# ICME-Lab/msm-webgpu

Measured on AMD Instinct MI355X. Metric: BN254 MSM/s at 2^20 points, higher is better.
Workload: dtype u32

## Files before the change

### include/msm_hip.h

```cpp
#ifndef MSM_HIP_H
#define MSM_HIP_H

#include <stddef.h>
#include <stdint.h>

#ifdef __cplusplus
extern "C" {
#endif

#define MSM_HIP_OK 0
#define MSM_HIP_ERR_NO_DEVICE (-1)
#define MSM_HIP_ERR_INVALID_ARG (-2)
#define MSM_HIP_ERR_OUT_OF_MEMORY (-3)
#define MSM_HIP_ERR_NONCANONICAL (-4)
#define MSM_HIP_ERR_NOT_ON_CURVE (-5)
#define MSM_HIP_ERR_NO_BASES (-6)
#define MSM_HIP_ERR_HIP (-7)
#define MSM_HIP_ERR_SLOT_BUSY (-8)

#define MSM_HIP_NUM_WINDOWS 16
#define MSM_HIP_WINDOW_BITS 16
#define MSM_HIP_MAX_LOCAL_WINDOWS 64
#define MSM_HIP_NUM_SLOTS 4
#define MSM_HIP_BUCKETS_PER_WINDOW 32768
// ... 103 lines not shown
int msm_hip_msm_bn254_g1(const uint8_t* xy_host, const uint8_t* scalars_host, size_t n, uint8_t out_xyz[96]);
int msm_hip_msm_curve(int curve, const uint8_t* xy_host, const uint8_t* scalars_host, size_t n, uint8_t* out_xyz);
void msm_hip_oneshot_release(void);

int msm_hip_sample_scalars_device(msm_hip_ctx* ctx, uint64_t seed, size_t n, void* scalars_dev);
int msm_hip_sample_points_device(msm_hip_ctx* ctx, uint64_t seed, size_t n, void* xy_dev);

int msm_hip_last_stage_ms(msm_hip_ctx* ctx, float* ms, int cap);
int msm_hip_set_stage_timing(msm_hip_ctx* ctx, int level);
void* msm_hip_stream(msm_hip_ctx* ctx);

#ifdef MSM_HIP_TEST_HOOKS
int msm_hip_set_debug(msm_hip_ctx* ctx, int keep_digit_planes);
int msm_hip_set_fine_hist_min_n(msm_hip_ctx* ctx, size_t n);
int msm_hip_test_skew_credit(const msm_hip_ctx* ctx);
int msm_hip_test_env_report(const msm_hip_ctx* ctx, char* out, size_t cap);
int msm_hip_read_digits(msm_hip_ctx* ctx, uint16_t* out, size_t cap_elems);
int msm_hip_read_col_ptr(msm_hip_ctx* ctx, uint32_t* out, size_t cap_elems);
int msm_hip_read_val_idxs(msm_hip_ctx* ctx, uint32_t* out, size_t cap_elems);
int msm_hip_read_buckets(msm_hip_ctx* ctx, uint8_t* out, size_t cap_bytes);
int msm_hip_read_window_sums(msm_hip_ctx* ctx, uint8_t* out, size_t cap_bytes);

int msm_hip_test_fq_op(msm_hip_ctx* ctx, int op, const uint8_t* a, const uint8_t* b, uint8_t* out, size_t n);
int msm_hip_test_g1_op(msm_hip_ctx* ctx, int op, const uint8_t* a, const uint8_t* b, uint8_t* out, size_t n);
int msm_hip_test_g1_mul_u32(msm_hip_ctx* ctx, const uint8_t* a, const uint32_t* k, uint8_t* out, size_t n);

int msm_hip_mgpu_inject_fault(msm_hip_mgpu* m, int device_index, int launches);

int msm_hip_test_oneshot_parts(int parts, size_t min_points);
#endif
// ... 33 lines not shown
```

### msm-webgpu_amd/api.py

```python
import ctypes as C
import os

import numpy as np
import torch

from . import build as _build

P = 21888242871839275222246405745257275088696311157297823662689037894645226208583
R_BN254 = 21888242871839275222246405745257275088548364400416034343698204186575808495617
PALLAS_P = 0x40000000000000000000000000000000224698fc094cf91b992d30ed00000001
VESTA_P = 0x40000000000000000000000000000000224698fc0994a8dd8c46eb2100000001
BLS12_381_P = 0x1a0111ea397fe69a4b1ba7b6434bacd764774b84f38512bf6730d2a0f6b0f6241eabfffeb153ffffb9feffffffffaaab
CURVES = {"bn254": (0, P), "grumpkin": (1, R_BN254), "pallas": (2, PALLAS_P), "vesta": (3, VESTA_P), "bls12_381": (4, BLS12_381_P),
          "bn254_g2": (5, P), "bls12_381_g2": (6, BLS12_381_P)}


def coord_bytes(curve):
    return {"bls12_381": 48, "bn254_g2": 64, "bls12_381_g2": 96}.get(curve, 32)
NUM_WINDOWS = 16
WINDOW_BITS = 16
BUCKETS_PER_WINDOW = 1 << 15

_lib = None

# ... 49 lines not shown
        L.msm_hip_slot_sync.argtypes = [vp, i]
        L.msm_hip_combine_windows_bn254.argtypes = [u8p, i, u8p]
        L.msm_hip_msm_bn254_g1.argtypes = [u8p, u8p, sz, u8p]
        L.msm_hip_msm_curve.argtypes = [i, u8p, u8p, sz, u8p]
        L.msm_hip_test_oneshot_parts.argtypes = [i, sz]
        L.msm_hip_oneshot_release.argtypes = []
        L.msm_hip_oneshot_release.restype = None
        L.msm_hip_sample_scalars_device.argtypes = [vp, C.c_uint64, sz, vp]
        L.msm_hip_sample_points_device.argtypes = [vp, C.c_uint64, sz, vp]
        L.msm_hip_last_stage_ms.argtypes = [vp, C.POINTER(C.c_float), i]
        L.msm_hip_stream.argtypes = [vp]
        L.msm_hip_stream.restype = vp
        L.msm_hip_set_debug.argtypes = [vp, i]
        L.msm_hip_set_fine_hist_min_n.argtypes = [vp, sz]
        L.msm_hip_test_skew_credit.argtypes = [vp]
        L.msm_hip_test_env_report.argtypes = [vp, C.c_char_p, sz]
        L.msm_hip_set_scalar_format.argtypes = [vp, C.c_uint32]
        L.msm_hip_set_stage_timing.argtypes = [vp, i]
        L.msm_hip_set_window_bits.argtypes = [vp, i]
        L.msm_hip_set_wide_bits.argtypes = [vp, i]
        L.msm_hip_wide_bits.argtypes = [vp]
        L.msm_hip_wide_config.argtypes = [i, i, C.c_size_t] + [C.POINTER(C.c_int)] * 4
        L.msm_hip_window_config.argtypes = [i, C.POINTER(i), C.POINTER(i)]
        L.msm_hip_last_window_bits.argtypes = [vp]
        L.msm_hip_endomorphism_window_count.argtypes = [i]
        L.msm_hip_uses_endomorphism.argtypes = [vp]
        L.msm_hip_batch_group_size.argtypes = [vp, sz]
        L.msm_hip_read_digits.argtypes = [vp, vp, sz]
        L.msm_hip_read_col_ptr.argtypes = [vp, vp, sz]
        L.msm_hip_read_val_idxs.argtypes = [vp, vp, sz]
# ... 455 lines not shown
        if mont256 and width != 32:
            raise ValueError("mont256 scalars are 32 bytes wide")
        fmt = SCALAR_WIDTHS[width] if width != 32 else (1 if mont256 else 0)
        _check(lib().msm_hip_set_scalar_format(self._h, fmt), "msm_hip_set_scalar_format")
        self.scalar_width = width

    def skew_credit(self):
        return lib().msm_hip_test_skew_credit(self._h)

    def env_report(self):
        return env_report(self._h)

    def set_fine_hist_min_n(self, n):
        _check(lib().msm_hip_set_fine_hist_min_n(self._h, n), "msm_hip_set_fine_hist_min_n")

    def set_debug(self, keep_digit_planes=True):
        _check(lib().msm_hip_set_debug(self._h, 1 if keep_digit_planes else 0), "msm_hip_set_debug")

    def read_digits(self, n, w_count=NUM_WINDOWS):
        a = np.empty((w_count, n), dtype=np.uint16)
        _check(lib().msm_hip_read_digits(self._h, a.ctypes.data, a.size), "msm_hip_read_digits")
        return a

    def read_col_ptr(self, w_count=NUM_WINDOWS, buckets=BUCKETS_PER_WINDOW):
        a = np.empty((w_count, buckets + 1), dtype=np.uint32)
        _check(lib().msm_hip_read_col_ptr(self._h, a.ctypes.data, a.size), "msm_hip_read_col_ptr")
        return a

    def read_val_idxs(self, n, w_count=NUM_WINDOWS):
        a = np.empty((w_count, n), dtype=np.uint32)
# ... 172 lines not shown
```

### msm-webgpu_amd/csrc/msm_hip.hip

```cpp
#include <hip/hip_runtime.h>
#include <hip/hip_ext.h>

#include <algorithm>
#include <chrono>
#include <cmath>
#include <cstdio>
#include <cstdlib>
#include <cstring>
#include <mutex>
#include <new>
#include <type_traits>

#define MSM_HIP_TEST_HOOKS 1
#include "../../include/msm_hip.h"
#include "curve_ops.h"
#include "host_pool.h"

#define MSM_FIELD_NS bn254
#define MSM_KERNEL_NS msmk
#define MSM_CURVE_CONSTANTS "bn254_constants.h"
#include "curve_unit.h"
#undef MSM_FIELD_NS
#undef MSM_KERNEL_NS
#undef MSM_CURVE_CONSTANTS
// ... 47 lines not shown
  bool pairs = false;
  uint32_t* sums_dev = nullptr;
  int wbits = WBITS;
  uint32_t half = 0, ncoarse = 0;
  int w_count = 0;
  int nwin = 0, combine_bits = 0;
  bool whole = false;
  size_t n_sc = 0, n_entries = 0;
  int full_windows = 0;
  bool digits = false;
  bool planes = false, share_shape = false, list_path = false;
  uint32_t tiles = 0, tile_len = 0, subtiles = 0;
  uint32_t chunks = 0, chunk_len = 0;
  size_t stride = 0;
  bool sparse = false;
  const uint32_t* indices = nullptr;
};

struct Slot {
  uint8_t* h_wsums = nullptr;
  uint8_t* d_wsums = nullptr;
  uint32_t* d_buckets = nullptr;
  size_t cap_buckets = 0;
  uint32_t* d_partials = nullptr;
  uint32_t* d_col_ptr = nullptr;
  uint32_t* d_heads = nullptr;
  uint32_t* d_tails = nullptr;
  uint32_t* d_big_queue = nullptr;
  hipEvent_t ev[N_MAIN_EVENTS] = {};
  hipEvent_t red0 = nullptr, red1 = nullptr;
// ... 69 lines not shown
  uint32_t* d_bin_total = nullptr;
  uint32_t* d_coarse_ptr = nullptr;
  uint32_t* d_tmp_val = nullptr;
  uint8_t* d_tmp_fine = nullptr;
  uint32_t* d_val = nullptr;
  uint32_t* d_chunk_slot = nullptr;
  uint32_t* d_list_len = nullptr;
  size_t cap_list_len = 0;
  uint32_t* d_scalar_conv = nullptr;
  size_t cap_scalar_conv = 0;
  uint32_t scalar_format = 0;
  int window_bits = 0;
  uint32_t* d_part_hist = nullptr;
  size_t fine_hist_min_n = FINE_BIG + 1;
  int skew_credit = 0;
  uint32_t* d_err = nullptr;
  uint8_t* d_stage = nullptr;
  size_t cap_stage = 0;

  Slot slot[NSLOT];
  LaunchPlan last;
  int last_slot = 0;
  int last_logr = 0;
  bool last_inline_reduce = false;
  bool last_fine_hist = false;
  bool sort_fine_hist = false;
  float stage_ms[10] = {};
};

namespace {
// ... 377 lines not shown
  p.tile_len = 2048;
  if ((p.n_sc + p.tile_len - 1) / p.tile_len > MAX_TILES) p.tile_len = (uint32_t)((((p.n_sc + MAX_TILES - 1) / MAX_TILES) + tile_unit - 1) / tile_unit * tile_unit);
  p.tiles = (uint32_t)((p.n_sc + p.tile_len - 1) / p.tile_len);
  p.subtiles = (uint32_t)((p.n_sc + LIST_SUB - 1) / LIST_SUB);
  if (wide) {
    const WideShape ws = wide_shape(n, ctx->curve, ctx->wide_bits, w_count);
    p.chunk_len = ws.host_len;
    p.chunks = ws.chunks;
  } else {
    p.chunk_len = chunk_len_for(p.n_entries, w_count);
    p.chunks = chunks_for(p.n_entries, p.chunk_len);
  }
  p.stride = stride_for(p.n_entries);
  p.sparse = sparse;
  p.indices = indices;
  return MSM_HIP_OK;
}

template <auto V0, auto... Vs, typename F>
void dispatch(decltype(V0) v, F&& f) {
  if constexpr (sizeof...(Vs) == 0) f(std::integral_constant<decltype(V0), V0>{});
  else if (v == V0) f(std::integral_constant<decltype(V0), V0>{});
  else dispatch<Vs...>(v, f);
}

int enqueue_sort(msm_hip_ctx* ctx, const LaunchPlan& p, Slot& s, const uint32_t* d_scalars) {
  const bool merge = p.mode == MODE_TABLES, halves = p.mode == MODE_HALVES, wide = p.mode == MODE_WIDE;
  const bool bytes = byte_windows(p.nb);
  const size_t merge_nb = merge || wide ? ctx->n_bases : 0;
  hipStream_t st = ctx->stream;
// ... 79 lines not shown
    });
  } else if (p.planes) {
    hipLaunchKernelGGL(k_scatter_planes, dim3(p.tiles), dim3(256), 0, st, ctx->d_digits, halves ? ctx->d_negbits : (const uint64_t*)nullptr, p.n_sc, p.stride,
                       p.tile_len, p.tiles, p.w_count, p.w_count_vec, ctx->d_counts, ctx->d_bin_total, ctx->d_coarse_ptr, ctx->d_tmp_val, ctx->d_tmp_fine,
                       (uint32_t)ctx->n_bases, p.chunks, p.chunk_len, d_chunk_len);
  } else if (bytes) {
    dispatch<1, 2>(p.nb, [&](auto b) {
      if (p.sparse)
        hipLaunchKernelGGL((k_byte_scatter<decltype(b)::value, SparseIdx>), grid, block, 0, st, (const uint8_t*)d_scalars, p.n, p.stride, p.tile_len, p.tiles,
                           p.w_count, ctx->d_counts, ctx->d_bin_total, s.d_col_ptr, p.half, ctx->d_val, p.chunks, p.chunk_len, d_chunk_len, sp);
      else
        hipLaunchKernelGGL(k_byte_scatter<decltype(b)::value>, grid, block, 0, st, (const uint8_t*)d_scalars, p.n, p.stride, p.tile_len, p.tiles, p.w_count,
                           ctx->d_counts, ctx->d_bin_total, s.d_col_ptr, p.half, ctx->d_val, p.chunks, p.chunk_len, d_chunk_len);
    });
  } else {
    dispatch<16, 14, 12>(p.wbits, [&](auto c) {
      dispatch<8, 4, 2, 1>(sw, [&](auto w) {
        constexpr int C = decltype(c)::value, SW = decltype(w)::value, NB = SW < 4 ? 4 * SW : 0;
        if (p.sparse)
          hipLaunchKernelGGL((k_scatter_coarse<C, SW, NB, SparseIdx>), grid, block, gpos_bytes, st, d_scalars, p.n_sc, p.stride, p.tile_len, p.tiles, p.w_begin,
                             p.w_count_vec, p.nvec, p.n * (NB ? NB : 8), ctx->d_counts, ctx->d_bin_total, ctx->d_coarse_ptr, ctx->d_tmp_val, ctx->d_tmp_fine,
                             merge_nb, (uint32_t)p.n, halves ? (uint32_t)ctx->n_bases : 0u, p.chunks, p.chunk_len, d_chunk_len, sp);
        else
          hipLaunchKernelGGL((k_scatter_coarse<C, SW, NB>), grid, block, gpos_bytes, st, d_scalars, p.n_sc, p.stride, p.tile_len, p.tiles, p.w_begin,
                             p.w_count_vec, p.nvec, p.n * (NB ? NB : 8), ctx->d_counts, ctx->d_bin_total, ctx->d_coarse_ptr, ctx->d_tmp_val, ctx->d_tmp_fine,
                             merge_nb, (uint32_t)p.n, halves ? (uint32_t)ctx->n_bases : 0u, p.chunks, p.chunk_len, d_chunk_len);
      });
    });
  }
  AFTER_KERNEL(ctx, "k_scatter_coarse", st);
  HIP_TRY(ctx, mark(3));
  if (bytes) {
    hipLaunchKernelGGL(k_byte_chunks, dim3(blocks_for(p.chunks, 256), p.w_count), dim3(256), 0, st, (const uint32_t*)s.d_col_ptr, p.half, p.chunks,
                       (const uint32_t*)d_chunk_len, ctx->d_chunk_slot);
    AFTER_KERNEL(ctx, "k_byte_chunks", st);
  } else {
    const uint32_t* part_hist = nullptr;
    const bool hist_useful = p.nb || ctx->fine_hist_min_n != FINE_BIG + 1 || p.n_entries / p.ncoarse * 4 > (size_t)FINE_BIG * 3 || ctx->skew_credit > 0;
    if (ctx->skew_credit > 0 && !p.nb) ctx->skew_credit--;
    ctx->sort_fine_hist = p.n_entries >= ctx->fine_hist_min_n && hist_useful;
    if (ctx->sort_fine_hist) {
      hipLaunchKernelGGL(k_fine_hist, dim3(p.ncoarse, p.w_count, FINE_SPLIT), dim3(256), 0, st, ctx->d_tmp_fine, p.stride, ctx->d_coarse_ptr,
                         ctx->d_part_hist);
      AFTER_KERNEL(ctx, "k_fine_hist", st);
      part_hist = ctx->d_part_hist;
    }
    hipLaunchKernelGGL(k_sort_fine, dim3(p.ncoarse, p.w_count, FINE_SPLIT), dim3(256), 0, st, ctx->d_tmp_val, ctx->d_tmp_fine, p.stride, ctx->d_coarse_ptr,
                       s.d_col_ptr, ctx->d_val, p.chunks, d_chunk_len, ctx->d_chunk_slot, part_hist, d_err);
    AFTER_KERNEL(ctx, "k_sort_fine", st);
  }
  if (ctx->debug) {
    hipLaunchKernelGGL(k_order_runs, dim3(blocks_for(p.n_entries, 256), p.w_count), dim3(256), 0, st, s.d_col_ptr, ctx->d_val, ctx->d_tmp_val, p.stride, p.half);
    hipLaunchKernelGGL(k_copy_runs, dim3(blocks_for(p.n_entries, 256), p.w_count), dim3(256), 0, st, s.d_col_ptr, ctx->d_tmp_val, ctx->d_val, p.stride, p.half);
    AFTER_KERNEL(ctx, "k_order_runs", st);
  }
  return MSM_HIP_OK;
}

struct RowCol {
  void (*kernel)(const uint32_t*, uint32_t*, uint32_t*);
  int blocks;
  int logr;
};
// ... 1012 lines not shown

int msm_hip_uses_endomorphism(const msm_hip_ctx* ctx) { return ctx ? (ctx->endo ? 1 : 0) : MSM_HIP_ERR_INVALID_ARG; }

int msm_hip_batch_group_size(msm_hip_ctx* ctx, size_t n) {
  if (!ctx) return MSM_HIP_ERR_INVALID_ARG;
  return (int)batch_group(ctx, n, (size_t)MAXLW);
}

int msm_hip_set_fine_hist_min_n(msm_hip_ctx* ctx, size_t n) {
  if (!ctx) return MSM_HIP_ERR_INVALID_ARG;
  ctx->fine_hist_min_n = n;
  return MSM_HIP_OK;
}

int msm_hip_test_skew_credit(const msm_hip_ctx* ctx) { return ctx ? ctx->skew_credit : MSM_HIP_ERR_INVALID_ARG; }

int msm_hip_test_env_report(const msm_hip_ctx* ctx, char* out, size_t cap) {
  if (!out || !cap) return MSM_HIP_ERR_INVALID_ARG;
  size_t len = 0;
  bool fits = true;
  auto put = [&](const char* key, long long v) {
    const int w = snprintf(out + len, cap - len, "%s=%lld\n", key, v);
    if (w < 0 || (size_t)w >= cap - len) fits = false;
    else len += (size_t)w;
  };
  put("target_lanes", (long long)target_lanes());
  put("chunk_search", chunk_search());
  put("window_bits", env_window_bits());
  put("bpr_logr", bpr_force_logr());
  put("planes_max_w", planes_max_w());
// ... 16 lines not shown
  put("upload_parts", g_probe_upload_parts.load());
  put("upload_chunks", g_probe_upload_chunks.load());
  if (ctx) {
    put("fine_hist_min_n", (long long)ctx->fine_hist_min_n);
    put("last_wbits", ctx->last.wbits);
    put("last_chunk_len", ctx->last.chunk_len);
    put("last_chunks", ctx->last.chunks);
    put("last_planes", ctx->last.planes);
    put("last_list_path", ctx->last.list_path);
    put("last_mode", ctx->last.mode);
    put("last_w_count", ctx->last.w_count);
    put("last_wide_top_shift", ctx->last.mode == MODE_WIDE ? wide_top_shift(ctx->curve, ctx->last.wide_bits) : 0);
    put("last_logr", ctx->last_logr);
    put("last_inline_reduce", ctx->last_inline_reduce);
    put("last_fine_hist", ctx->last_fine_hist);
  }
  return fits ? (int)len : MSM_HIP_ERR_INVALID_ARG;
}

int msm_hip_set_debug(msm_hip_ctx* ctx, int keep_digit_planes) {
  if (!ctx) return MSM_HIP_ERR_INVALID_ARG;
  ctx->debug = keep_digit_planes != 0;
  return MSM_HIP_OK;
}

int msm_hip_read_digits(msm_hip_ctx* ctx, uint16_t* out, size_t cap_elems) {
  if (!ctx || !ctx->last.digits) return MSM_HIP_ERR_INVALID_ARG;
  return read_back(ctx, out, ctx->d_digits, ctx->last.n_sc * ctx->last.w_count * 2, cap_elems * 2);
}
int msm_hip_read_col_ptr(msm_hip_ctx* ctx, uint32_t* out, size_t cap_elems) {
// ... 154 lines not shown
```

### msm-webgpu_amd/csrc/msm_kernels.h

```cpp
#ifndef MSM_CURVE_UNIT
#pragma once
#include "g1.h"
#endif
#include <hip/hip_runtime.h>

#include <utility>

#ifndef MSM_SPARSE_IDX
#define MSM_SPARSE_IDX
struct SparseIdx {
  const uint32_t* idx;
  uint32_t n_bases;
  uint32_t* err;
};
#endif

namespace MSM_KERNEL_NS {
using namespace MSM_FIELD_NS;

constexpr int WBITS = 16;
constexpr int NWIN = 16;
constexpr int MAXLW = 64;
constexpr int HALF = 1 << (WBITS - 1);
constexpr int CW = FQ_WORDS;
// ... 198 lines not shown
  for (int w = 1; w < num_tables; w++) {
    const int steps = w == num_tables - 1 ? last_step_bits : step_bits;
#pragma unroll 1
    for (int k = 0; k < steps; k++) acc = g1_double(acc);
    const fq t = fq_inv(fq_mul(acc.zz, acc.zzz));
    const fq x = fq_canonical(fq_mul(acc.x, fq_mul(t, acc.zzz)));
    const fq y = fq_canonical(fq_mul(acc.y, fq_mul(t, acc.zz)));
    st_fq(bases + ((size_t)w * nb + i) * PT_WORDS, x);
    st_fq(bases + ((size_t)w * nb + i) * PT_WORDS + CW, y);
    acc = g1_from_affine(x, y);
  }
}

constexpr int NCOARSE = 128;
constexpr int FINE = HALF / NCOARSE;

template <int C, int SW = 8, int NB = 0>
__host__ __device__ constexpr uint32_t bias_word(int i) {
  uint32_t v = 0;
  for (int w = 0; w < WinCfg<C, SW, NB>::NWIN; w++) {
    const int bit = C * w + C - 1;
    if (bit / 32 == i) v |= 1u << (bit % 32);
  }
  return v;
}
template <int C, int SW = 8, int NB = 0>
__device__ __forceinline__ uint32_t bias_scalar(const uint32_t s[SW], uint32_t t[WinCfg<C, SW, NB>::WORDS]) {
  constexpr int WORDS = WinCfg<C, SW, NB>::WORDS;
  uint64_t c = 0;
#pragma unroll
// ... 91 lines not shown
}

__global__ void __launch_bounds__(256) k_scalars_from_mont256(const uint32_t* __restrict__ in, uint32_t* __restrict__ out, size_t count,
                                                              uint32_t* __restrict__ err) {
  const size_t i = (size_t)blockIdx.x * blockDim.x + threadIdx.x;
  if (i >= count) return;
  uint32_t w[8], o[8];
  ld8(in + i * 8, w);
  if (geq_modulus<1>(w)) atomicOr(err, ERRBIT_NONCANONICAL);
  fr_from_mont256(w, o);
  uint4* q = reinterpret_cast<uint4*>(out + i * 8);
  q[0] = make_uint4(o[0], o[1], o[2], o[3]);
  q[1] = make_uint4(o[4], o[5], o[6], o[7]);
}

__device__ __forceinline__ SparseIdx sparse_arg() { return SparseIdx{nullptr, 0u, nullptr}; }
__device__ __forceinline__ SparseIdx sparse_arg(SparseIdx s) { return s; }
template <int C, int SW, bool SPLIT = false, int NB = 0, typename... Sparse>
__global__ void __launch_bounds__(256) k_count(const uint32_t* __restrict__ scalars, size_t n, uint32_t tile_len, uint32_t tiles,
                                               int w_begin, int w_count, int nvec, size_t vec_stride,
                                               uint32_t* __restrict__ counts, uint16_t* __restrict__ planes, int plane_mode,
                                               uint64_t* __restrict__ negbits, uint32_t* __restrict__ halves_out,
                                               uint32_t* __restrict__ err, size_t merge_nb, Sparse... sparse) {
  static_assert(!SPLIT || SW == 4, "the split produces 4-word halves");
  static_assert(!SPLIT || NB == 0, "narrow scalars are never split");
  constexpr bool SPARSE = sizeof...(Sparse) != 0;
  const SparseIdx sp = sparse_arg(sparse...);
  uint32_t bad_idx = 0;
  __shared__ uint32_t cnt[MAXLW * NCOARSE];
  const int tid = threadIdx.x;
  const int v = blockIdx.y;
  const int le0 = merge_nb ? v : v * w_count, le_n = merge_nb ? 1 : w_count;
  (void)nvec;
  for (int i = tid; i < le_n * NCOARSE; i += 256) cnt[le0 * NCOARSE + i] = 0;
// ... 5 lines not shown
#pragma unroll
    for (int w = 0; w < WinCfg<C, SW, NB>::NWIN; w++) {
      const int lw = w - w_begin;
      if (lw >= 0 && lw < w_count) {
        const int le = merge_nb ? v : v * w_count + lw;
        const uint32_t code = code_of_window<C>(tb, w);
        if (code != 0) atomicAdd(&cnt[le * NCOARSE + ((code & 0x7fffu) >> 8)], 1u);
        if (plane_mode) planes[((size_t)v * w_count + lw) * n + pos] = (uint16_t)(plane_mode == 2 ? code : (code ? code ^ (neg << 15) : 0u));
      }
    }
  };
  {
    const uint32_t* sv = scalars + (size_t)v * vec_stride;
    if constexpr (SPLIT) {
      const size_t nsc = n / 2, neg_words = (nsc + 63) / 64;
      for (size_t j0 = base / 2; j0 < end / 2; j0 += 256) {
        const size_t j = j0 + tid;
        const bool valid = j < end / 2;
        uint32_t k[8], h[2][4];
#pragma unroll
        for (int q = 0; q < 8; q++) k[q] = 0;
        bool live = valid;
        if constexpr (SPARSE) {
          if (valid && sp.idx[j] >= sp.n_bases) live = false, bad_idx = 1;
        }
        if (live) ld8(sv + j * 8, k);
        uint64_t c = 0;
#pragma unroll
        for (int q = 0; q < 8; q++) c = (c + k[q] + 0x80008000u) >> 32;
        const bool ok = glv_split(k, h[0], h[1]);
        if (c != 0 || !ok) bad = 1;
        if (negbits) {
#pragma unroll
          for (int hh = 0; hh < 2; hh++) {
            const unsigned long long nb = __ballot((h[hh][3] >> 31) != 0u);
            if ((tid & 63) == 0 && valid) negbits[((size_t)v * 2 + hh) * neg_words + j / 64] = nb;
          }
        }
        if (!valid) continue;
        if (halves_out) {
          uint4* o = reinterpret_cast<uint4*>(halves_out + ((size_t)v * nsc + j) * 8);
          o[0] = make_uint4(h[0][0], h[0][1], h[0][2], h[0][3]);
          o[1] = make_uint4(h[1][0], h[1][1], h[1][2], h[1][3]);
        }
#pragma unroll
        for (int hh = 0; hh < 2; hh++) {
          uint32_t s[4] = {h[hh][0], h[hh][1], h[hh][2], h[hh][3] & 0x7fffffffu}, tb[WinCfg<C, 4>::WORDS];
          bad |= bias_scalar<C, 4>(s, tb);
          emit(v, 2 * j + hh, tb, h[hh][3] >> 31);
        }
      }
    } else if constexpr (NB != 0) {
      const uint8_t* nv = reinterpret_cast<const uint8_t*>(scalars) + (size_t)v * vec_stride;
      for (size_t i0 = base; i0 < end; i0 += 256) {
        const size_t i = i0 + tid;
        if (i >= end) continue;
        uint32_t s[SW], tb[WinCfg<C, SW, NB>::WORDS];
        ld_narrow<NB>(nv, i, s);
        if constexpr (SPARSE) {
          if (sp.idx[i] >= sp.n_bases) {
            bad_idx = 1;
#pragma unroll
            for (int k = 0; k < SW; k++) s[k] = 0;
          }
// ... 21 lines not shown
          bad |= bias_scalar<16>(s, t16);
        }
        emit(v, i, tb, neg);
      }
    }
  }
  if (bad) atomicOr(err, ERRBIT_SCALAR_CARRY);
  if constexpr (SPARSE) {
    if (bad_idx) atomicOr(err, ERRBIT_BAD_INDEX);
  }
  __syncthreads();
  for (int i = tid; i < le_n * NCOARSE; i += 256)
    counts[((size_t)(le0 + i / NCOARSE) * tiles + blockIdx.x) * NCOARSE + (i % NCOARSE)] = cnt[le0 * NCOARSE + i];
}

__global__ void __launch_bounds__(256) k_scan_tiles(uint32_t* __restrict__ counts, uint32_t tiles, uint32_t* __restrict__ bin_total) {
  const int lw = blockIdx.y, lane = threadIdx.x & 63;
  const int bin = blockIdx.x * 4 + (threadIdx.x >> 6);
  uint32_t* c = counts + (size_t)lw * tiles * NCOARSE + bin;
  uint32_t run = 0;
  for (uint32_t t0 = 0; t0 < tiles; t0 += 64) {
    const uint32_t t = t0 + lane;
    const uint32_t v = t < tiles ? c[(size_t)t * NCOARSE] : 0u;
    uint32_t x = v;
#pragma unroll
    for (int off = 1; off < 64; off <<= 1) {
      const uint32_t y = __shfl_up(x, off);
      if (lane >= off) x += y;
    }
    if (t < tiles) c[(size_t)t * NCOARSE] = run + x - v;
    run += __shfl(x, 63);
  }
  if (lane == 0) bin_total[lw * NCOARSE + bin] = run;
}

__device__ __forceinline__ uint32_t block_excl_scan_256(uint32_t v, uint32_t* wave_tot) {
  const int lane = threadIdx.x & 63, wid = threadIdx.x >> 6;
  uint32_t x = v;
#pragma unroll
  for (int off = 1; off < 64; off <<= 1) {
    const uint32_t y = __shfl_up(x, off);
    if (lane >= off) x += y;
  }
  if (lane == 63) wave_tot[wid] = x;
  __syncthreads();
// ... 109 lines not shown
      __syncthreads();
      const uint32_t mine = tid < NCOARSE ? hist[tid] : 0u;
      const uint32_t excl = block_excl_scan_256(mine, wave_tot);
      if (tid < NCOARSE) lstart[tid] = excl;
      __syncthreads();
      const uint32_t total = lstart[NCOARSE - 1] + hist[NCOARSE - 1];
#pragma unroll
      for (int j = 0; j < PER; j++) {
        const uint32_t code = code_of_window<C>(sc[j], w);
        if (code) {
          const uint32_t slot = code & 0x7fffu, bin = slot >> 8;
          const uint32_t e = lstart[bin] + rank[j];
          uint32_t pos = (uint32_t)(sub + (size_t)j * 256 + tid);
          if constexpr (SPARSE) pos = rec[j];
          else if constexpr (SW == 4) pos = (pos >> 1) + ((pos & 1u) ? half_shift : 0u);
          st_val[e] = (idx_base + pos) | (((code >> 15) ^ ((negs >> j) & 1u)) << 31);
          st_fine[e] = (uint8_t)(slot & 0xffu);
          st_dst[e] = gpos[lw * NCOARSE + bin] + rank[j];
        }
      }
      __syncthreads();
      uint32_t* ov = tmp_val + (size_t)lw * stride;
      uint8_t* of = tmp_fine + (size_t)lw * stride;
      for (uint32_t e = tid; e < total; e += 256) {
        const uint32_t d = st_dst[e];
        ov[d] = st_val[e];
        of[d] = st_fine[e];
      }
      if (tid < NCOARSE) gpos[lw * NCOARSE + tid] += hist[tid];
      __syncthreads();
    }
  }
}

constexpr int BYTE_BINS = 256;
constexpr int BYTE_MAXLW = MAXLW * NCOARSE / BYTE_BINS;
template <int NB>
__device__ __forceinline__ uint32_t ld_byte_scalar(const uint8_t* v, size_t i) {
  static_assert(NB == 1 || NB == 2, "byte windows: U8 / U16");
  if constexpr (NB == 1) return v[i];
  else return reinterpret_cast<const uint16_t*>(v)[i];
}
// ... 750 lines not shown
  const unsigned long long vm = __ballot(valid);
  if (vm == 0) return;
  const int first = __ffsll((long long)vm) - 1;
  const uint32_t k0 = (uint32_t)__builtin_amdgcn_readlane((int)key, first);
  const bool same = valid && key == k0;
  const unsigned long long sm = __ballot(same);
  if ((int)(threadIdx.x & 63) == first) atomicAdd(&counter[k0], (uint32_t)__popcll(sm));
  if (valid && !same) atomicAdd(&counter[key], 1u);
}

constexpr int FINE_SPLIT = 8;

constexpr uint32_t FINE_BIG = 32768;
static_assert(FINE_BIG % FINE_CHUNK == 0, "sub-ranges are whole chunks");

__global__ void __launch_bounds__(256) k_fine_hist(const uint8_t* __restrict__ tmp_fine, size_t stride,
                                                   const uint32_t* __restrict__ coarse_ptr, uint32_t* __restrict__ part_hist) {
  __shared__ uint32_t hist[FINE];
  const int bin = blockIdx.x, part = blockIdx.z, lw = blockIdx.y, tid = threadIdx.x;
  const uint32_t begin = coarse_ptr[(size_t)lw * (NCOARSE + 1) + bin], end = coarse_ptr[(size_t)lw * (NCOARSE + 1) + bin + 1];
  if (end - begin <= FINE_BIG) return;
  uint32_t per = (end - begin + FINE_SPLIT - 1) / FINE_SPLIT;
  per = (per + FINE_CHUNK - 1) / FINE_CHUNK * FINE_CHUNK;
  const uint32_t my_begin = begin + (uint32_t)part * per < end ? begin + (uint32_t)part * per : end;
  const uint32_t my_end = my_begin + per < end ? my_begin + per : end;
  const uint8_t* tf = tmp_fine + (size_t)lw * stride;
  hist[tid] = 0;
  __syncthreads();
  for (uint32_t base = my_begin; base < my_end; base += FINE_CHUNK) {
    uint32_t f[FINE_PER];
#pragma unroll
    for (int j = 0; j < FINE_PER; j++) {
      const uint32_t i = base + j * 256 + tid;
      f[j] = i < my_end ? tf[i] : 0xffffffffu;
    }
#pragma unroll
    for (int j = 0; j < FINE_PER; j++) lds_count_only(hist, f[j] & 0xffu, f[j] != 0xffffffffu);
  }
  __syncthreads();
  part_hist[(((size_t)lw * NCOARSE + bin) * FINE_SPLIT + part) * FINE + tid] = hist[tid];
}

__global__ void __launch_bounds__(256) k_sort_fine(const uint32_t* __restrict__ tmp_val, const uint8_t* __restrict__ tmp_fine, size_t stride,
                                                   const uint32_t* __restrict__ coarse_ptr, uint32_t* __restrict__ col_ptr,
                                                   uint32_t* __restrict__ val_idxs, uint32_t chunks, const uint32_t* __restrict__ chunk_len_dev,
                                                   uint32_t* __restrict__ chunk_slot, const uint32_t* __restrict__ part_hist, uint32_t* __restrict__ info) {
  const uint32_t chunk_len = *chunk_len_dev;
  __shared__ uint32_t hist[FINE];
  __shared__ uint32_t before[FINE];
  __shared__ uint32_t lstart[FINE];
  __shared__ uint32_t gpos[FINE];
  __shared__ uint32_t wave_tot[4];
  __shared__ uint32_t st_val[FINE_CHUNK];
  __shared__ uint8_t st_slot[FINE_CHUNK];
  __shared__ uint32_t long_c0[FINE], long_c1[FINE], long_slot[FINE];
  __shared__ uint32_t skew_flag, long_count;
  const int bin = blockIdx.x, part = blockIdx.z, lw = blockIdx.y, tid = threadIdx.x;
  const uint32_t half = gridDim.x * FINE;
  const uint32_t begin = coarse_ptr[(size_t)lw * (NCOARSE + 1) + bin], end = coarse_ptr[(size_t)lw * (NCOARSE + 1) + bin + 1];
  const bool big = end - begin > FINE_BIG;
  if (!big && part != 0) return;
  uint32_t my_begin = begin, my_end = end;
  if (big) {
    uint32_t per = (end - begin + FINE_SPLIT - 1) / FINE_SPLIT;
    per = (per + FINE_CHUNK - 1) / FINE_CHUNK * FINE_CHUNK;
    my_begin = begin + (uint32_t)part * per < end ? begin + (uint32_t)part * per : end;
    my_end = my_begin + per < end ? my_begin + per : end;
  }
  const uint32_t* tv = tmp_val + (size_t)lw * stride;
  const uint8_t* tf = tmp_fine + (size_t)lw * stride;
  uint32_t* out = val_idxs + (size_t)lw * stride;
  hist[tid] = 0;
  before[tid] = 0;
  if (tid == 0) {
    skew_flag = 0;
    long_count = 0;
  }
  __syncthreads();
  if (!big) {
    for (uint32_t base = begin; base < end; base += FINE_CHUNK) {
      uint32_t f[FINE_PER];
#pragma unroll
      for (int j = 0; j < FINE_PER; j++) {
        const uint32_t i = base + j * 256 + tid;
        f[j] = i < end ? tf[i] : 0xffffffffu;
      }
#pragma unroll
      for (int j = 0; j < FINE_PER; j++)
        if (f[j] != 0xffffffffu) atomicAdd(&hist[f[j]], 1u);
    }
  } else if (part_hist) {
    if (tid == 0 && part == 0) atomicOr(info, INFOBIT_HUGE_BIN);
    const uint32_t* ph = part_hist + ((size_t)lw * NCOARSE + bin) * FINE_SPLIT * FINE + tid;
    uint32_t all = 0, front = 0;
#pragma unroll
    for (int q = 0; q < FINE_SPLIT; q++) {
      const uint32_t c = ph[q * FINE];
      all += c;
      if (q < part) front += c;
    }
    hist[tid] = all;
    before[tid] = front;
  } else {
    if (tid == 0 && part == 0) atomicOr(info, INFOBIT_HUGE_BIN);
    uint32_t f[FINE_PER], g[FINE_PER];
#pragma unroll
    for (int j = 0; j < FINE_PER; j++) {
      const uint32_t i = begin + j * 256 + tid;
      f[j] = i < end ? tf[i] : 0xffffffffu;
    }
    for (uint32_t base = begin; base < end; base += FINE_CHUNK) {
#pragma unroll
      for (int j = 0; j < FINE_PER; j++) {
        const uint32_t i = base + FINE_CHUNK + j * 256 + tid;
        g[j] = i < end ? tf[i] : 0xffffffffu;
      }
      uint32_t* counter = base < my_begin ? before : hist;
#pragma unroll
      for (int j = 0; j < FINE_PER; j++) lds_count_only(counter, f[j] & 0xffu, f[j] != 0xffffffffu);
#pragma unroll
      for (int j = 0; j < FINE_PER; j++) f[j] = g[j];
    }
    __syncthreads();
    hist[tid] += before[tid];
  }
  __syncthreads();
  if (hist[tid] > (end - begin) / 4 && end - begin > (uint32_t)FINE_CHUNK) skew_flag = 1;
  {
    const uint32_t excl = block_excl_scan_256(hist[tid], wave_tot);
    gpos[tid] = begin + excl + before[tid];
// ... 20 lines not shown
  {
    const uint32_t nl = long_count, nparts = big ? FINE_SPLIT : 1;
    for (uint32_t k = 0; k < nl; k++)
      for (uint32_t c = long_c0[k] + part * 256 + tid; c < long_c1[k]; c += nparts * 256) chunk_slot[(size_t)lw * chunks + c] = long_slot[k];
  }
  __syncthreads();
  const bool skewed = skew_flag != 0;
  for (uint32_t base = my_begin; base < my_end; base += FINE_CHUNK) {
    hist[tid] = 0;
    __syncthreads();
    uint32_t v[FINE_PER], fr[FINE_PER];
#pragma unroll
    for (int j = 0; j < FINE_PER; j++) {
      const uint32_t i = base + j * 256 + tid;
      const bool valid = i < my_end;
      const uint32_t f = valid ? tf[i] : 0u;
      const uint32_t rank = skewed ? lds_count_rank(hist, f, valid) : (valid ? atomicAdd(&hist[f], 1u) : 0u);
      if (valid) {
        v[j] = tv[i];
        fr[j] = f | (rank << 8);
      } else {
        fr[j] = 0xffffffffu;
      }
    }
    __syncthreads();
    const uint32_t excl = block_excl_scan_256(hist[tid], wave_tot);
    lstart[tid] = excl;
    __syncthreads();
    const uint32_t total = (my_end - base) < (uint32_t)FINE_CHUNK ? (my_end - base) : (uint32_t)FINE_CHUNK;
#pragma unroll
    for (int j = 0; j < FINE_PER; j++) {
      if (fr[j] != 0xffffffffu) {
        const uint32_t f = fr[j] & 0xffu, r = fr[j] >> 8;
        const uint32_t e = lstart[f] + r;
// ... 1011 lines not shown
```

Baseline: 736.5.

## Pack fine bucket key into value word; prefetch in split count and scan

```diff
diff --git a/include/msm_hip.h b/include/msm_hip.h
--- a/include/msm_hip.h
+++ b/include/msm_hip.h
@@ -141,6 +141,7 @@
 int msm_hip_set_debug(msm_hip_ctx* ctx, int keep_digit_planes);
 int msm_hip_set_fine_hist_min_n(msm_hip_ctx* ctx, size_t n);
 int msm_hip_test_skew_credit(const msm_hip_ctx* ctx);
+int msm_hip_test_pack_fine(msm_hip_ctx* ctx, int allow);
 int msm_hip_test_env_report(const msm_hip_ctx* ctx, char* out, size_t cap);
 int msm_hip_read_digits(msm_hip_ctx* ctx, uint16_t* out, size_t cap_elems);
 int msm_hip_read_col_ptr(msm_hip_ctx* ctx, uint32_t* out, size_t cap_elems);
diff --git a/msm-webgpu_amd/api.py b/msm-webgpu_amd/api.py
--- a/msm-webgpu_amd/api.py
+++ b/msm-webgpu_amd/api.py
@@ -87,6 +87,7 @@
         L.msm_hip_set_debug.argtypes = [vp, i]
         L.msm_hip_set_fine_hist_min_n.argtypes = [vp, sz]
         L.msm_hip_test_skew_credit.argtypes = [vp]
+        L.msm_hip_test_pack_fine.argtypes = [vp, i]
         L.msm_hip_test_env_report.argtypes = [vp, C.c_char_p, sz]
         L.msm_hip_set_scalar_format.argtypes = [vp, C.c_uint32]
         L.msm_hip_set_stage_timing.argtypes = [vp, i]
@@ -572,6 +573,9 @@
     def set_fine_hist_min_n(self, n):
         _check(lib().msm_hip_set_fine_hist_min_n(self._h, n), "msm_hip_set_fine_hist_min_n")
 
+    def set_pack_fine(self, allow=True):
+        _check(lib().msm_hip_test_pack_fine(self._h, 1 if allow else 0), "msm_hip_test_pack_fine")
+
     def set_debug(self, keep_digit_planes=True):
         _check(lib().msm_hip_set_debug(self._h, 1 if keep_digit_planes else 0), "msm_hip_set_debug")
 
diff --git a/msm-webgpu_amd/csrc/msm_hip.hip b/msm-webgpu_amd/csrc/msm_hip.hip
--- a/msm-webgpu_amd/csrc/msm_hip.hip
+++ b/msm-webgpu_amd/csrc/msm_hip.hip
@@ -85,6 +85,7 @@
   uint32_t chunks = 0, chunk_len = 0;
   size_t stride = 0;
   bool sparse = false;
+  bool packed = false;
   const uint32_t* indices = nullptr;
 };
 
@@ -184,6 +185,7 @@
   uint32_t* d_part_hist = nullptr;
   size_t fine_hist_min_n = FINE_BIG + 1;
   int skew_credit = 0;
+  bool pack_fine = true;
   uint32_t* d_err = nullptr;
   uint8_t* d_stage = nullptr;
   size_t cap_stage = 0;
@@ -591,6 +593,8 @@
   p.stride = stride_for(p.n_entries);
   p.sparse = sparse;
   p.indices = indices;
+  const size_t rec_bound = merge ? (size_t)(w_begin + w_count_vec) * ctx->n_bases : halves ? 2 * ctx->n_bases : ctx->n_bases;
+  p.packed = ctx->pack_fine && !wide && !p.planes && !byte_windows(nb) && rec_bound <= ((size_t)1 << FINE_KEY_SHIFT);
   return MSM_HIP_OK;
 }
 
@@ -700,16 +704,17 @@
                            ctx->d_counts, ctx->d_bin_total, s.d_col_ptr, p.half, ctx->d_val, p.chunks, p.chunk_len, d_chunk_len);
     });
   } else {
+    uint8_t* tmp_fine = p.packed ? nullptr : ctx->d_tmp_fine;
     dispatch<16, 14, 12>(p.wbits, [&](auto c) {
       dispatch<8, 4, 2, 1>(sw, [&](auto w) {
         constexpr int C = decltype(c)::value, SW = decltype(w)::value, NB = SW < 4 ? 4 * SW : 0;
         if (p.sparse)
           hipLaunchKernelGGL((k_scatter_coarse<C, SW, NB, SparseIdx>), grid, block, gpos_bytes, st, d_scalars, p.n_sc, p.stride, p.tile_len, p.tiles, p.w_begin,
-                             p.w_count_vec, p.nvec, p.n * (NB ? NB : 8), ctx->d_counts, ctx->d_bin_total, ctx->d_coarse_ptr, ctx->d_tmp_val, ctx->d_tmp_fine,
+                             p.w_count_vec, p.nvec, p.n * (NB ? NB : 8), ctx->d_counts, ctx->d_bin_total, ctx->d_coarse_ptr, ctx->d_tmp_val, tmp_fine,
                              merge_nb, (uint32_t)p.n, halves ? (uint32_t)ctx->n_bases : 0u, p.chunks, p.chunk_len, d_chunk_len, sp);
         else
           hipLaunchKernelGGL((k_scatter_coarse<C, SW, NB>), grid, block, gpos_bytes, st, d_scalars, p.n_sc, p.stride, p.tile_len, p.tiles, p.w_begin,
-                             p.w_count_vec, p.nvec, p.n * (NB ? NB : 8), ctx->d_counts, ctx->d_bin_total, ctx->d_coarse_ptr, ctx->d_tmp_val, ctx->d_tmp_fine,
+                             p.w_count_vec, p.nvec, p.n * (NB ? NB : 8), ctx->d_counts, ctx->d_bin_total, ctx->d_coarse_ptr, ctx->d_tmp_val, tmp_fine,
                              merge_nb, (uint32_t)p.n, halves ? (uint32_t)ctx->n_bases : 0u, p.chunks, p.chunk_len, d_chunk_len);
       });
     });
@@ -726,13 +731,14 @@
     if (ctx->skew_credit > 0 && !p.nb) ctx->skew_credit--;
     ctx->sort_fine_hist = p.n_entries >= ctx->fine_hist_min_n && hist_useful;
     if (ctx->sort_fine_hist) {
-      hipLaunchKernelGGL(k_fine_hist, dim3(p.ncoarse, p.w_count, FINE_SPLIT), dim3(256), 0, st, ctx->d_tmp_fine, p.stride, ctx->d_coarse_ptr,
-                         ctx->d_part_hist);
+      hipLaunchKernelGGL(p.packed ? k_fine_hist<true> : k_fine_hist<false>, dim3(p.ncoarse, p.w_count, FINE_SPLIT), dim3(256), 0, st,
+                         (const uint32_t*)ctx->d_tmp_val, (const uint8_t*)ctx->d_tmp_fine, p.stride, (const uint32_t*)ctx->d_coarse_ptr, ctx->d_part_hist);
       AFTER_KERNEL(ctx, "k_fine_hist", st);
       part_hist = ctx->d_part_hist;
     }
-    hipLaunchKernelGGL(k_sort_fine, dim3(p.ncoarse, p.w_count, FINE_SPLIT), dim3(256), 0, st, ctx->d_tmp_val, ctx->d_tmp_fine, p.stride, ctx->d_coarse_ptr,
-                       s.d_col_ptr, ctx->d_val, p.chunks, d_chunk_len, ctx->d_chunk_slot, part_hist, d_err);
+    hipLaunchKernelGGL(p.packed ? k_sort_fine<true> : k_sort_fine<false>, dim3(p.ncoarse, p.w_count, FINE_SPLIT), dim3(256), 0, st,
+                       (const uint32_t*)ctx->d_tmp_val, (const uint8_t*)ctx->d_tmp_fine, p.stride, (const uint32_t*)ctx->d_coarse_ptr, s.d_col_ptr, ctx->d_val,
+                       p.chunks, (const uint32_t*)d_chunk_len, ctx->d_chunk_slot, part_hist, d_err);
     AFTER_KERNEL(ctx, "k_sort_fine", st);
   }
   if (ctx->debug) {
@@ -1775,6 +1781,12 @@
 }
 
 int msm_hip_test_skew_credit(const msm_hip_ctx* ctx) { return ctx ? ctx->skew_credit : MSM_HIP_ERR_INVALID_ARG; }
+
+int msm_hip_test_pack_fine(msm_hip_ctx* ctx, int allow) {
+  if (!ctx) return MSM_HIP_ERR_INVALID_ARG;
+  ctx->pack_fine = allow != 0;
+  return MSM_HIP_OK;
+}
 
 int msm_hip_test_env_report(const msm_hip_ctx* ctx, char* out, size_t cap) {
   if (!out || !cap) return MSM_HIP_ERR_INVALID_ARG;
@@ -1821,6 +1833,7 @@
     put("last_logr", ctx->last_logr);
     put("last_inline_reduce", ctx->last_inline_reduce);
     put("last_fine_hist", ctx->last_fine_hist);
+    put("last_packed_fine", ctx->last.packed);
   }
   return fits ? (int)len : MSM_HIP_ERR_INVALID_ARG;
 }
diff --git a/msm-webgpu_amd/csrc/msm_kernels.h b/msm-webgpu_amd/csrc/msm_kernels.h
--- a/msm-webgpu_amd/csrc/msm_kernels.h
+++ b/msm-webgpu_amd/csrc/msm_kernels.h
@@ -236,6 +236,8 @@
 
 constexpr int NCOARSE = 128;
 constexpr int FINE = HALF / NCOARSE;
+constexpr int FINE_KEY_SHIFT = 23;
+constexpr uint32_t FINE_KEY_MASK = 0xffu << FINE_KEY_SHIFT;
 
 template <int C, int SW = 8, int NB = 0>
 __host__ __device__ constexpr uint32_t bias_word(int i) {
@@ -357,10 +359,14 @@
   q[1] = make_uint4(o[4], o[5], o[6], o[7]);
 }
 
+#ifndef MSM_COUNT_SPLIT_PF
+#define MSM_COUNT_SPLIT_PF 2
+#endif
+constexpr int COUNT_SPLIT_PF = MSM_COUNT_SPLIT_PF;
 __device__ __forceinline__ SparseIdx sparse_arg() { return SparseIdx{nullptr, 0u, nullptr}; }
 __device__ __forceinline__ SparseIdx sparse_arg(SparseIdx s) { return s; }
 template <int C, int SW, bool SPLIT = false, int NB = 0, typename... Sparse>
-__global__ void __launch_bounds__(256) k_count(const uint32_t* __restrict__ scalars, size_t n, uint32_t tile_len, uint32_t tiles,
+__global__ void __launch_bounds__(256, SPLIT ? 4 : 1) k_count(const uint32_t* __restrict__ scalars, size_t n, uint32_t tile_len, uint32_t tiles,
                                                int w_begin, int w_count, int nvec, size_t vec_stride,
                                                uint32_t* __restrict__ counts, uint16_t* __restrict__ planes, int plane_mode,
                                                uint64_t* __restrict__ negbits, uint32_t* __restrict__ halves_out,
@@ -396,40 +402,50 @@
     const uint32_t* sv = scalars + (size_t)v * vec_stride;
     if constexpr (SPLIT) {
       const size_t nsc = n / 2, neg_words = (nsc + 63) / 64;
-      for (size_t j0 = base / 2; j0 < end / 2; j0 += 256) {
-        const size_t j = j0 + tid;
-        const bool valid = j < end / 2;
-        uint32_t k[8], h[2][4];
-#pragma unroll
-        for (int q = 0; q < 8; q++) k[q] = 0;
-        bool live = valid;
-        if constexpr (SPARSE) {
-          if (valid && sp.idx[j] >= sp.n_bases) live = false, bad_idx = 1;
+      for (size_t j00 = base / 2; j00 < end / 2; j00 += 256 * COUNT_SPLIT_PF) {
+        uint32_t kk[COUNT_SPLIT_PF][8];
+#pragma unroll
+        for (int u = 0; u < COUNT_SPLIT_PF; u++) {
+          const size_t j = j00 + (size_t)u * 256 + tid;
+#pragma unroll
+          for (int q = 0; q < 8; q++) kk[u][q] = 0;
+          bool live = j < end / 2;
+          if constexpr (SPARSE) {
+            if (live && sp.idx[j] >= sp.n_bases) live = false, bad_idx = 1;
+          }
+          if (live) ld8(sv + j * 8, kk[u]);
         }
-        if (live) ld8(sv + j * 8, k);
-        uint64_t c = 0;
-#pragma unroll
-        for (int q = 0; q < 8; q++) c = (c + k[q] + 0x80008000u) >> 32;
-        const bool ok = glv_split(k, h[0], h[1]);
-        if (c != 0 || !ok) bad = 1;
-        if (negbits) {
+#pragma unroll
+        for (int u = 0; u < COUNT_SPLIT_PF; u++) {
+          const size_t j = j00 + (size_t)u * 256 + tid;
+          if (j00 + (size_t)u * 256 >= end / 2) break;
+          const bool valid = j < end / 2;
+          const uint32_t* k = kk[u];
+          uint32_t h[2][4];
+          uint64_t c = 0;
+#pragma unroll
+          for (int q = 0; q < 8; q++) c = (c + k[q] + 0x80008000u) >> 32;
+          const bool ok = glv_split(k, h[0], h[1]);
+          if (c != 0 || !ok) bad = 1;
+          if (negbits) {
+#pragma unroll
+            for (int hh = 0; hh < 2; hh++) {
+              const unsigned long long nb = __ballot((h[hh][3] >> 31) != 0u);
+              if ((tid & 63) == 0 && valid) negbits[((size_t)v * 2 + hh) * neg_words + j / 64] = nb;
+            }
+          }
+          if (!valid) continue;
+          if (halves_out) {
+            uint4* o = reinterpret_cast<uint4*>(halves_out + ((size_t)v * nsc + j) * 8);
+            o[0] = make_uint4(h[0][0], h[0][1], h[0][2], h[0][3]);
+            o[1] = make_uint4(h[1][0], h[1][1], h[1][2], h[1][3]);
+          }
 #pragma unroll
           for (int hh = 0; hh < 2; hh++) {
-            const unsigned long long nb = __ballot((h[hh][3] >> 31) != 0u);
-            if ((tid & 63) == 0 && valid) negbits[((size_t)v * 2 + hh) * neg_words + j / 64] = nb;
+            uint32_t s[4] = {h[hh][0], h[hh][1], h[hh][2], h[hh][3] & 0x7fffffffu}, tb[WinCfg<C, 4>::WORDS];
+            bad |= bias_scalar<C, 4>(s, tb);
+            emit(v, 2 * j + hh, tb, h[hh][3] >> 31);
           }
-        }
-        if (!valid) continue;
-        if (halves_out) {
-          uint4* o = reinterpret_cast<uint4*>(halves_out + ((size_t)v * nsc + j) * 8);
-          o[0] = make_uint4(h[0][0], h[0][1], h[0][2], h[0][3]);
-          o[1] = make_uint4(h[1][0], h[1][1], h[1][2], h[1][3]);
-        }
-#pragma unroll
-        for (int hh = 0; hh < 2; hh++) {
-          uint32_t s[4] = {h[hh][0], h[hh][1], h[hh][2], h[hh][3] & 0x7fffffffu}, tb[WinCfg<C, 4>::WORDS];
-          bad |= bias_scalar<C, 4>(s, tb);
-          emit(v, 2 * j + hh, tb, h[hh][3] >> 31);
         }
       }
     } else if constexpr (NB != 0) {
@@ -481,21 +497,31 @@
     counts[((size_t)(le0 + i / NCOARSE) * tiles + blockIdx.x) * NCOARSE + (i % NCOARSE)] = cnt[le0 * NCOARSE + i];
 }
 
+constexpr int SCAN_PER = 16;
 __global__ void __launch_bounds__(256) k_scan_tiles(uint32_t* __restrict__ counts, uint32_t tiles, uint32_t* __restrict__ bin_total) {
   const int lw = blockIdx.y, lane = threadIdx.x & 63;
   const int bin = blockIdx.x * 4 + (threadIdx.x >> 6);
   uint32_t* c = counts + (size_t)lw * tiles * NCOARSE + bin;
   uint32_t run = 0;
-  for (uint32_t t0 = 0; t0 < tiles; t0 += 64) {
-    const uint32_t t = t0 + lane;
-    const uint32_t v = t < tiles ? c[(size_t)t * NCOARSE] : 0u;
-    uint32_t x = v;
+  for (uint32_t t0 = 0; t0 < tiles; t0 += 64 * SCAN_PER) {
+    const uint32_t tb = t0 + (uint32_t)lane * SCAN_PER;
+    uint32_t v[SCAN_PER], s = 0;
+#pragma unroll
+    for (int k = 0; k < SCAN_PER; k++) v[k] = tb + k < tiles ? c[(size_t)(tb + k) * NCOARSE] : 0u;
+#pragma unroll
+    for (int k = 0; k < SCAN_PER; k++) s += v[k];
+    uint32_t x = s;
 #pragma unroll
     for (int off = 1; off < 64; off <<= 1) {
       const uint32_t y = __shfl_up(x, off);
       if (lane >= off) x += y;
     }
-    if (t < tiles) c[(size_t)t * NCOARSE] = run + x - v;
+    uint32_t acc = run + x - s;
+#pragma unroll
+    for (int k = 0; k < SCAN_PER; k++) {
+      if (tb + k < tiles) c[(size_t)(tb + k) * NCOARSE] = acc;
+      acc += v[k];
+    }
     run += __shfl(x, 63);
   }
   if (lane == 0) bin_total[lw * NCOARSE + bin] = run;
@@ -635,18 +661,22 @@
           uint32_t pos = (uint32_t)(sub + (size_t)j * 256 + tid);
           if constexpr (SPARSE) pos = rec[j];
           else if constexpr (SW == 4) pos = (pos >> 1) + ((pos & 1u) ? half_shift : 0u);
-          st_val[e] = (idx_base + pos) | (((code >> 15) ^ ((negs >> j) & 1u)) << 31);
+          st_val[e] = (idx_base + pos) | (((code >> 15) ^ ((negs >> j) & 1u)) << 31) | (tmp_fine ? 0u : (slot & 0xffu) << FINE_KEY_SHIFT);
           st_fine[e] = (uint8_t)(slot & 0xffu);
           st_dst[e] = gpos[lw * NCOARSE + bin] + rank[j];
         }
       }
       __syncthreads();
       uint32_t* ov = tmp_val + (size_t)lw * stride;
-      uint8_t* of = tmp_fine + (size_t)lw * stride;
-      for (uint32_t e = tid; e < total; e += 256) {
-        const uint32_t d = st_dst[e];
-        ov[d] = st_val[e];
-        of[d] = st_fine[e];
+      if (tmp_fine) {
+        uint8_t* of = tmp_fine + (size_t)lw * stride;
+        for (uint32_t e = tid; e < total; e += 256) {
+          const uint32_t d = st_dst[e];
+          ov[d] = st_val[e];
+          of[d] = st_fine[e];
+        }
+      } else {
+        for (uint32_t e = tid; e < total; e += 256) ov[st_dst[e]] = st_val[e];
       }
       if (tid < NCOARSE) gpos[lw * NCOARSE + tid] += hist[tid];
       __syncthreads();
@@ -1427,7 +1457,13 @@
 constexpr uint32_t FINE_BIG = 32768;
 static_assert(FINE_BIG % FINE_CHUNK == 0, "sub-ranges are whole chunks");
 
-__global__ void __launch_bounds__(256) k_fine_hist(const uint8_t* __restrict__ tmp_fine, size_t stride,
+template <bool PACKED>
+__device__ __forceinline__ uint32_t fine_key(const uint32_t* tv, const uint8_t* tf, uint32_t i) {
+  if constexpr (PACKED) return (tv[i] >> FINE_KEY_SHIFT) & 0xffu;
+  else return tf[i];
+}
+template <bool PACKED>
+__global__ void __launch_bounds__(256) k_fine_hist(const uint32_t* __restrict__ tmp_val, const uint8_t* __restrict__ tmp_fine, size_t stride,
                                                    const uint32_t* __restrict__ coarse_ptr, uint32_t* __restrict__ part_hist) {
   __shared__ uint32_t hist[FINE];
   const int bin = blockIdx.x, part = blockIdx.z, lw = blockIdx.y, tid = threadIdx.x;
@@ -1437,7 +1473,8 @@
   per = (per + FINE_CHUNK - 1) / FINE_CHUNK * FINE_CHUNK;
   const uint32_t my_begin = begin + (uint32_t)part * per < end ? begin + (uint32_t)part * per : end;
   const uint32_t my_end = my_begin + per < end ? my_begin + per : end;
-  const uint8_t* tf = tmp_fine + (size_t)lw * stride;
+  const uint32_t* tv = tmp_val + (size_t)lw * stride;
+  const uint8_t* tf = PACKED ? nullptr : tmp_fine + (size_t)lw * stride;
   hist[tid] = 0;
   __syncthreads();
   for (uint32_t base = my_begin; base < my_end; base += FINE_CHUNK) {
@@ -1445,7 +1482,7 @@
 #pragma unroll
     for (int j = 0; j < FINE_PER; j++) {
       const uint32_t i = base + j * 256 + tid;
-      f[j] = i < my_end ? tf[i] : 0xffffffffu;
+      f[j] = i < my_end ? fine_key<PACKED>(tv, tf, i) : 0xffffffffu;
     }
 #pragma unroll
     for (int j = 0; j < FINE_PER; j++) lds_count_only(hist, f[j] & 0xffu, f[j] != 0xffffffffu);
@@ -1454,6 +1491,7 @@
   part_hist[(((size_t)lw * NCOARSE + bin) * FINE_SPLIT + part) * FINE + tid] = hist[tid];
 }
 
+template <bool PACKED>
 __global__ void __launch_bounds__(256) k_sort_fine(const uint32_t* __restrict__ tmp_val, const uint8_t* __restrict__ tmp_fine, size_t stride,
                                                    const uint32_t* __restrict__ coarse_ptr, uint32_t* __restrict__ col_ptr,
                                                    uint32_t* __restrict__ val_idxs, uint32_t chunks, const uint32_t* __restrict__ chunk_len_dev,
@@ -1481,7 +1519,7 @@
     my_end = my_begin + per < end ? my_begin + per : end;
   }
   const uint32_t* tv = tmp_val + (size_t)lw * stride;
-  const uint8_t* tf = tmp_fine + (size_t)lw * stride;
+  const uint8_t* tf = PACKED ? nullptr : tmp_fine + (size_t)lw * stride;
   uint32_t* out = val_idxs + (size_t)lw * stride;
   hist[tid] = 0;
   before[tid] = 0;
@@ -1496,7 +1534,7 @@
 #pragma unroll
       for (int j = 0; j < FINE_PER; j++) {
         const uint32_t i = base + j * 256 + tid;
-        f[j] = i < end ? tf[i] : 0xffffffffu;
+        f[j] = i < end ? fine_key<PACKED>(tv, tf, i) : 0xffffffffu;
       }
 #pragma unroll
       for (int j = 0; j < FINE_PER; j++)
@@ -1520,13 +1558,13 @@
 #pragma unroll
     for (int j = 0; j < FINE_PER; j++) {
       const uint32_t i = begin + j * 256 + tid;
-      f[j] = i < end ? tf[i] : 0xffffffffu;
+      f[j] = i < end ? fine_key<PACKED>(tv, tf, i) : 0xffffffffu;
     }
     for (uint32_t base = begin; base < end; base += FINE_CHUNK) {
 #pragma unroll
       for (int j = 0; j < FINE_PER; j++) {
         const uint32_t i = base + FINE_CHUNK + j * 256 + tid;
-        g[j] = i < end ? tf[i] : 0xffffffffu;
+        g[j] = i < end ? fine_key<PACKED>(tv, tf, i) : 0xffffffffu;
       }
       uint32_t* counter = base < my_begin ? before : hist;
 #pragma unroll
@@ -1577,10 +1615,11 @@
     for (int j = 0; j < FINE_PER; j++) {
       const uint32_t i = base + j * 256 + tid;
       const bool valid = i < my_end;
-      const uint32_t f = valid ? tf[i] : 0u;
+      const uint32_t w = PACKED && valid ? tv[i] : 0u;
+      const uint32_t f = !valid ? 0u : PACKED ? (w >> FINE_KEY_SHIFT) & 0xffu : tf[i];
       const uint32_t rank = skewed ? lds_count_rank(hist, f, valid) : (valid ? atomicAdd(&hist[f], 1u) : 0u);
       if (valid) {
-        v[j] = tv[i];
+        v[j] = PACKED ? w & ~FINE_KEY_MASK : tv[i];
         fr[j] = f | (rank << 8);
       } else {
         fr[j] = 0xffffffffu;
```

New measurement: 728.5 (median of 3 runs). Within noise of the previous version (-1.1%).
